# apollozkp/zkp-subnet

Measured on AMD Instinct MI355X. Metric: BLS12-381 G1 MSM points/sec at 2^20, higher is better.
Workload: dtype u32; 1 GPU; 2^20-point BLS12-381 G1 Pippenger MSM per GPU (uniform scalars in [0,r), cached SRS); points_per_gpu=1048576, window_bits=20, windows=13, buckets=524288, entries_per_lane=104, lanes=131072, requests_in_flight=1, world_size=1, parallelism=single GPU

## Files before the change

zkp_subnet_amd/csrc/msm.hip.h:

```cpp
#pragma once
#include "g1.hip.h"

struct WinLayout {
    int nwin;
    uint16_t off[66];
};
struct MsmShape {
    int c;
    int nwin;
    WinLayout lay;
    uint32_t nbuckets;
    uint64_t n;
    int nbatch;
    uint64_t srs_offset;
    uint64_t srs_stride;
    int chunk;
};

struct SortTail {
    uint32_t chunk;
    g1_xyzz_t* buckets;
    uint32_t* pin_dst;
    uint32_t* seq_word;
    uint32_t seq;
};
void launch_msm_sort(hipStream_t s, const MsmShape& sh, const uint32_t* scalars, int scalars_mont,
                     const uint32_t* scalars2, int scalars2_mont, uint32_t* part_ws, bool part_ws_clean, uint2* parted,
                     uint32_t* offsets, uint32_t* sorted, uint32_t* max_len_word, bool fast, uint32_t* overflow_word,
                     const SortTail* tail = nullptr);
bool msm_sort_fast_ok(const MsmShape& sh);
uint64_t msm_sort_parted_entries(const MsmShape& sh, bool fast);
void launch_publish(hipStream_t s, const void* src_dev, void* dst_host_devptr, uint32_t bytes, uint32_t* clear2 = nullptr,
                    uint32_t* seq_word_devptr = nullptr, uint32_t seq = 0);
void launch_msm_accumulate(hipStream_t s, const MsmShape& sh, const g1_affine_t* table, const uint32_t* offsets,
                           const uint32_t* sorted, g1_xyzz_t* buckets, g1_xyzz_t* carries, uint32_t* carry_key,
                           uint32_t nchunks);
void launch_fold_maxlen(hipStream_t s, const uint32_t* offsets, uint32_t nbuckets, uint32_t chunk, uint32_t* max_len,
                        g1_xyzz_t* buckets);
bool msm_fold_bucket_ok(uint32_t nbuckets, uint32_t max_run);
void launch_fold_bucket(hipStream_t s, const uint32_t* offsets, uint32_t chunk, uint32_t nbuckets, const g1_xyzz_t* carries,
                        g1_xyzz_t* buckets);
void launch_fold_step(hipStream_t s, const uint32_t* offsets, const uint32_t* carry_key, uint32_t chunk,
                      uint32_t nchunks, uint32_t d, g1_xyzz_t* carries);
void launch_fold_heads(hipStream_t s, const uint32_t* offsets, const uint32_t* carry_key, uint32_t chunk,
                       uint32_t nchunks, const g1_xyzz_t* carries, g1_xyzz_t* buckets);
void launch_msm_tree_level(hipStream_t s, const g1_xyzz_t* in, const g1_xyzz_t* prev, g1_xyzz_t* out,
                           uint32_t n_in_nodes, int level);
bool msm_tree_level2_ok(uint32_t n_in_nodes, int level);
void launch_msm_tree_level2(hipStream_t s, const g1_xyzz_t* in, const g1_xyzz_t* prev, g1_xyzz_t* mid_p, g1_xyzz_t* out,
                            uint32_t n_in_nodes, int level);
void launch_msm_final(hipStream_t s, const g1_xyzz_t* node, const g1_xyzz_t* prev, int nbits, int nodes,
                      g1_xyzz_t* out_xyzz, g1_xyzz_t* scratch);
void launch_g1_sum(hipStream_t s, const g1_xyzz_t* in, uint32_t count, g1_xyzz_t* out_xyzz);
void launch_g1_sum_affine(hipStream_t s, const g1_affine_t* in, uint32_t count, g1_xyzz_t* out_xyzz);
void launch_g1_subgroup_check(hipStream_t s, const g1_affine_t* in, uint32_t count, uint32_t* bad_flag);
void launch_g1_subgroup_check_bulk(hipStream_t s, const g1_affine_t* in, uint64_t n, uint32_t* bad_flag);
void launch_g1_compress(hipStream_t s, const g1_xyzz_t* in, uint8_t* out48);
void launch_g1_compress_pair(hipStream_t s, const g1_xyzz_t* in0, const g1_xyzz_t* in1, uint8_t* out0, uint8_t* out1);
void launch_xyzz_pack(hipStream_t s, const g1_xyzz_t* in, uint32_t* out48w, uint32_t count);
void launch_xyzz_unpack(hipStream_t s, const uint32_t* in48w, g1_xyzz_t* out, uint32_t count);

void launch_srs_from_be96(hipStream_t s, const uint8_t* be96, g1_affine_t* out, uint64_t n, uint32_t* bad_flag);
void launch_srs_from_c48(hipStream_t s, const uint8_t* c48, g1_affine_t* out, uint64_t n, uint32_t* bad_flag);
void launch_srs_to_c48(hipStream_t s, const g1_affine_t* in, uint8_t* c48, uint64_t n);
void launch_srs_to_be96(hipStream_t s, const g1_affine_t* in, uint8_t* be96, uint64_t n);
void launch_srs_precompute(hipStream_t s, g1_affine_t* table, uint64_t stride, uint64_t first, uint64_t count,
                           const WinLayout& lay, g1_xyzz_t* tmp);
void launch_srs_generate(hipStream_t s, g1_affine_t* out, uint64_t count, uint64_t j_base, const uint32_t* tau_mont,
                         const uint32_t* s0_mont, g1_affine_t* gtab, g1_xyzz_t* tmp, bool build_gtab);
```

zkp_subnet_amd/csrc/msm_tree.hip:

```cpp
#include "msm_dev.hip.h"

KZG_DEV void tree_operands(const g1_xyzz_t* in, const g1_xyzz_t* prev, uint32_t n_in, int level, uint32_t k, uint32_t m,
                           const g1_xyzz_t*& pa, const g1_xyzz_t*& pb) {
    if (level >= 1 && k == (uint32_t)level) {
        pa = &prev[4 * (uint64_t)m + 1];
        pb = &prev[4 * (uint64_t)m + 3];
    } else {
        pa = &in[(uint64_t)k * n_in + 2 * m];
        pb = pa + 1;
    }
}
#ifndef KZG_TREE_MIN_WAVES
#define KZG_TREE_MIN_WAVES 2
#endif
__global__ void __launch_bounds__(256, KZG_TREE_MIN_WAVES) k_msm_tree_level(const g1_xyzz_t* __restrict__ in,
                                                         const g1_xyzz_t* __restrict__ prev,
                                                         g1_xyzz_t* __restrict__ out, uint32_t n_in, int level) {
    tail_priority();
    const uint32_t n_out = n_in >> 1;
    const uint32_t gid = blockIdx.x * blockDim.x + threadIdx.x;
    if (gid >= n_out * (uint32_t)(level + 1)) return;
    const uint32_t k = gid / n_out, m = gid - k * n_out;
    const g1_xyzz_t *pa, *pb;
    tree_operands(in, prev, n_in, level, k, m, pa, pb);
    g1_xyzz_t a, b, r;
    load_xyzz(a, pa);
    load_xyzz(b, pb);
    g1_add<true>(r, a, b);
    if ((n_out & 63u) == 0) {
        __shared__ uint4 stage[4][64 * 15];
        const uint32_t lane = threadIdx.x & 63u;
        uint4* mine = stage[threadIdx.x >> 6];
        uint32_t t[56];
        const fp_t* f[4] = {&r.x, &r.y, &r.zz, &r.zzz};
#pragma unroll
        for (int c = 0; c < 4; c++)
#pragma unroll
            for (int i = 0; i < 14; i++) t[14 * c + i] = f[c]->l[i];
#pragma unroll
        for (int i = 0; i < 14; i++) mine[lane * 15 + i] = make_uint4(t[4 * i], t[4 * i + 1], t[4 * i + 2], t[4 * i + 3]);
        __builtin_amdgcn_fence(__ATOMIC_RELEASE, "wavefront");
        __builtin_amdgcn_wave_barrier();
        __builtin_amdgcn_fence(__ATOMIC_ACQUIRE, "wavefront");
        uint4* wb = reinterpret_cast<uint4*>(&out[(uint64_t)k * n_out + (m - lane)]);
#pragma unroll
        for (int i = 0; i < 14; i++) {
            const uint32_t g = (uint32_t)i * 64u + lane;
            const uint32_t pt = g / 14u;
            wb[g] = mine[pt * 15 + (g - pt * 14u)];
        }
        return;
    }
    store_xyzz(&out[(uint64_t)k * n_out + m], r);
}


__global__ void __launch_bounds__(256) k_msm_tree_level_coop(const g1_xyzz_t* __restrict__ in,
                                                              const g1_xyzz_t* __restrict__ prev,
                                                              g1_xyzz_t* __restrict__ out, uint32_t n_in, int level) {
    tail_priority();
    __shared__ CoopLds sm;
    const uint32_t n_out = n_in >> 1;
    const uint32_t gid = blockIdx.x * 64 + (threadIdx.x & 63);
    const bool active = gid < n_out * (uint32_t)(level + 1);
    const uint32_t k = active ? gid / n_out : 0, m = active ? gid - k * n_out : 0;
    const g1_xyzz_t *pa, *pb;
    tree_operands(in, prev, n_in, level, k, m, pa, pb);
    coop_add(sm, &out[(uint64_t)k * n_out + m], pa, pb, active);
}

__global__ void __launch_bounds__(64) k_msm_tree_level_lp(const g1_xyzz_t* __restrict__ in,
                                                           const g1_xyzz_t* __restrict__ prev,
                                                           g1_xyzz_t* __restrict__ out, uint32_t n_in, int level) {
    tail_priority();
    __shared__ LpScratch sm;
    const LpLane k = lp_lane();
    const uint32_t n_out = n_in >> 1;
    const uint32_t gid = blockIdx.x;
    const uint32_t c = gid / n_out, m = gid - c * n_out;
    const g1_xyzz_t *pa, *pb;
    tree_operands(in, prev, n_in, level, c, m, pa, pb);
    lp_add(sm, &out[(uint64_t)c * n_out + m], pa, pb, k);
}
__global__ void __launch_bounds__(128) k_msm_tree_level2_lp(const g1_xyzz_t* __restrict__ in,
                                                             const g1_xyzz_t* __restrict__ prev,
                                                             g1_xyzz_t* __restrict__ mid_p, g1_xyzz_t* __restrict__ out,
                                                             uint32_t n_in, int level) {
    tail_priority();
    __shared__ LpScratch sm[2];
    __shared__ __align__(16) g1_xyzz_t mid[2];
    const LpLane k = lp_lane();
    const uint32_t w = __builtin_amdgcn_readfirstlane(threadIdx.x >> 6);
    const uint32_t n2 = n_in >> 2;
    const uint32_t c = blockIdx.x / n2, j = blockIdx.x - c * n2;
    const bool late = c == (uint32_t)level + 1u;
    g1_xyzz_t* dst = &out[(uint64_t)c * n2 + j];
    if (late) {
        if (w == 0) lp_add(sm[0], dst, &in[4 * (uint64_t)j + 1], &in[4 * (uint64_t)j + 3], k);
    } else {
        const g1_xyzz_t *pa, *pb;
        tree_operands(in, prev, n_in, level, c, 2 * j + w, pa, pb);
        lp_add(sm[w], &mid[w], pa, pb, k);
    }
    __syncthreads();
    if (late) return;
    if (c == 0 && threadIdx.x < 112)
        reinterpret_cast<uint32_t*>(&mid_p[2 * (uint64_t)j])[threadIdx.x] = reinterpret_cast<const uint32_t*>(mid)[threadIdx.x];
    if (w == 0) lp_add(sm[0], dst, &mid[0], &mid[1], k);
}
#define FINAL_PTS 32
__global__ void __launch_bounds__(64) k_msm_final_dbl_lp(const g1_xyzz_t* __restrict__ node,
                                                          const g1_xyzz_t* __restrict__ prev, int nbits, int nodes,
                                                          g1_xyzz_t* __restrict__ pts) {
    tail_priority();
    __shared__ LpScratch sm;
    __shared__ g1_xyzz_t v;
    const LpLane k = lp_lane();
    const int l = (int)(blockIdx.x % (uint32_t)(nbits + 1));
    const uint32_t m = blockIdx.x / (uint32_t)(nbits + 1);
    const g1_xyzz_t* src = l < nbits - 1 ? &node[(uint64_t)(1 + l) * nodes + m] : l == nbits - 1 ? &prev[2 * m + 1] : &node[m];
    if (threadIdx.x < 56) reinterpret_cast<uint32_t*>(&v)[threadIdx.x] = reinterpret_cast<const uint32_t*>(src)[threadIdx.x];
    __syncthreads();
    if (l < nbits)
        for (int s = 0; s < l; s++) lp_dbl(sm, &v, &v, k);
    __syncthreads();
    if (threadIdx.x < 56)
        reinterpret_cast<uint32_t*>(&pts[(uint64_t)m * FINAL_PTS + l])[threadIdx.x] = reinterpret_cast<const uint32_t*>(&v)[threadIdx.x];
}
__global__ void __launch_bounds__(512) k_msm_final_sum_lp(const g1_xyzz_t* __restrict__ pts_g, int nbits,
                                                           g1_xyzz_t* __restrict__ out) {
    tail_priority();
    __shared__ LpScratch sm[8];
    __shared__ g1_xyzz_t pts[FINAL_PTS];
    const LpLane k = lp_lane();
    const int w = (int)__builtin_amdgcn_readfirstlane(threadIdx.x >> 6);
    const uint32_t m = blockIdx.x;
    const int count = nbits + 1;
    for (uint32_t i = threadIdx.x; i < (uint32_t)count * 56; i += 512)
        reinterpret_cast<uint32_t*>(pts)[i] = reinterpret_cast<const uint32_t*>(pts_g + (uint64_t)m * FINAL_PTS)[i];
    __syncthreads();
    for (int d = 16; d >= 1; d >>= 1) {
        for (int l = w; l < d; l += 8)
            if (l + d < count) lp_add(sm[w], &pts[l], &pts[l], &pts[l + d], k);
        __syncthreads();
    }
    if (threadIdx.x < 56) reinterpret_cast<uint32_t*>(&out[m])[threadIdx.x] = reinterpret_cast<const uint32_t*>(&pts[0])[threadIdx.x];
}


__global__ void __launch_bounds__(256) k_msm_final(const g1_xyzz_t* __restrict__ node,
                                                    const g1_xyzz_t* __restrict__ prev, int nbits, int nodes,
                                                    g1_xyzz_t* __restrict__ out) {
    tail_priority();
    __shared__ CoopLds sm;
    __shared__ g1_xyzz_t pts[64];
    const uint32_t l = threadIdx.x & 63;
    const uint32_t m = blockIdx.x;
    if (threadIdx.x < 64) {
        g1_xyzz_t v;
        g1_set_inf(v);
        if ((int)l < nbits - 1) load_xyzz(v, &node[(uint64_t)(1 + l) * nodes + m]);
        else if ((int)l == nbits - 1) load_xyzz(v, &prev[2 * m + 1]);
        else if ((int)l == nbits) load_xyzz(v, &node[m]);
        store_xyzz(&pts[l], v);
    }
    __syncthreads();
    for (int step = 0; step < nbits - 1; step++)
        coop_dbl(sm, &pts[l], &pts[l], (int)l < nbits && step < (int)l);
    for (uint32_t d = (nbits + 1 <= 32 ? 16 : 32); d >= 1; d >>= 1)
        coop_add(sm, &pts[l], &pts[l], &pts[l + d < 64 ? l + d : l], l < d);
    if (threadIdx.x == 0) {
        g1_xyzz_t v;
        load_xyzz(v, &pts[0]);
        store_xyzz(&out[m], v);
    }
}


#ifndef KZG_TREE_WIDE_MIN
#define KZG_TREE_WIDE_MIN 32768
#endif
void launch_msm_tree_level(hipStream_t s, const g1_xyzz_t* in, const g1_xyzz_t* prev, g1_xyzz_t* out,
                           uint32_t n_in_nodes, int level) {
    uint32_t ops = (n_in_nodes >> 1) * (uint32_t)(level + 1);
    if (ops > KZG_TREE_WIDE_MIN) k_msm_tree_level<<<nblk(ops, 256), 256, 0, s>>>(in, prev, out, n_in_nodes, level);
#ifndef KZG_NO_LP
    else if (ops <= LP_MAX_OPS) k_msm_tree_level_lp<<<ops, 64, 0, s>>>(in, prev, out, n_in_nodes, level);
#endif
    else k_msm_tree_level_coop<<<nblk(ops, 64), 256, 0, s>>>(in, prev, out, n_in_nodes, level);
}
bool msm_tree_level2_ok(uint32_t n_in_nodes, int level) {
#if defined(KZG_NO_LP) || defined(KZG_NO_TREE_PAIRS)
    (void)n_in_nodes; (void)level;
    return false;
#else
    return n_in_nodes >= 4 && (n_in_nodes >> 1) * (uint32_t)(level + 1) <= LP_MAX_OPS;
#endif
}
void launch_msm_tree_level2(hipStream_t s, const g1_xyzz_t* in, const g1_xyzz_t* prev, g1_xyzz_t* mid_p, g1_xyzz_t* out,
                            uint32_t n_in_nodes, int level) {
    k_msm_tree_level2_lp<<<(n_in_nodes >> 2) * (uint32_t)(level + 2), 128, 0, s>>>(in, prev, mid_p, out, n_in_nodes, level);
}
void launch_msm_final(hipStream_t s, const g1_xyzz_t* node, const g1_xyzz_t* prev, int nbits, int nodes,
                      g1_xyzz_t* out_xyzz, g1_xyzz_t* scratch) {
#ifndef KZG_NO_LP
    k_msm_final_dbl_lp<<<nodes * (nbits + 1), 64, 0, s>>>(node, prev, nbits, nodes, scratch);
    k_msm_final_sum_lp<<<nodes, 512, 0, s>>>(scratch, nbits, out_xyzz);
#else
    (void)scratch;
    k_msm_final<<<nodes, 256, 0, s>>>(node, prev, nbits, nodes, out_xyzz);
#endif
}
```

zkp_subnet_amd/csrc/pipeline.hip:

```cpp
#include "ctx.hip.h"

using namespace kzg_impl;

namespace kzg_impl {

#ifndef KZG_MIN_CHUNK
#define KZG_MIN_CHUNK 6
#endif
int pick_chunk(uint64_t entries) {
    const uint64_t lanes = 131072;
    if (entries <= lanes * 16) {
        const uint64_t k = (entries + lanes / 2 - 1) / (lanes / 2);
        return (int)(k < KZG_MIN_CHUNK ? KZG_MIN_CHUNK : k);
    }
    const uint64_t rounds = (entries + lanes * 512 - 1) / (lanes * 512);
    const uint64_t k = (entries + lanes * rounds - 1) / (lanes * rounds);
    return (int)k;
}
struct TreeBufs {
    g1_xyzz_t *in, *prev, *out, *extra;
};
static void run_tree(hipStream_t s, TreeBufs& b, uint32_t n_in, uint32_t stop) {
    for (int level = 0; n_in > stop;) {
        if ((n_in >> 2) >= stop && msm_tree_level2_ok(n_in, level)) {
            launch_msm_tree_level2(s, b.in, b.prev, b.out, b.extra, n_in, level);
            g1_xyzz_t *old_in = b.in, *old_prev = b.prev;
            b.in = b.extra;
            b.prev = b.out;
            b.out = old_prev;
            b.extra = old_in;
            level += 2;
            n_in >>= 2;
            continue;
        }
        launch_msm_tree_level(s, b.in, b.prev, b.out, n_in, level);
        g1_xyzz_t* recycled = b.prev;
        b.prev = b.in;
        b.in = b.out;
        b.out = recycled;
        level++;
        n_in >>= 1;
    }
}
int msm_core(kzg_ctx* ctx, Lane& L, const uint32_t* scalars, int mont, uint64_t n, uint64_t srs_offset,
             g1_xyzz_t* out_xyzz, const uint32_t* scalars2, int mont2) {
    hipStream_t s = L.stream;
    const int nbatch = scalars2 ? 2 : 1;
    if (n == 0) {
        HIPCHK(ctx, hipMemsetAsync(out_xyzz, 0, nbatch * sizeof(g1_xyzz_t), s));
        return KZG_OK;
    }
    if (srs_offset + n > ctx->stride) return fail(ctx, KZG_E_ARG, "MSM range exceeds the resident SRS");
    const uint64_t entries = n * (uint64_t)ctx->nwin * nbatch;
    if (entries >= ((uint64_t)1 << 32)) return fail(ctx, KZG_E_ARG, "MSM too large for 32-bit entry indices");
    MsmShape sh;
    sh.c = ctx->c; sh.nwin = ctx->nwin; sh.lay = ctx->lay; sh.nbuckets = ctx->nbuckets * nbatch; sh.n = n;
    sh.nbatch = nbatch;
    sh.srs_offset = srs_offset; sh.srs_stride = ctx->stride; sh.chunk = pick_chunk(entries);
    const uint32_t nchunks = (uint32_t)((entries + sh.chunk - 1) / sh.chunk);
    const size_t B = sh.nbuckets;
    L.expect_short = entries <= ((uint64_t)1 << 24);
    L.expect_us += 400 + (uint32_t)(entries / 4096);
    bool fast = msm_sort_fast_ok(sh) && L.skew_hint == 0;
    if (L.skew_hint > 0) L.skew_hint--;
    HIPCHK(ctx, L.rank.ensure(msm_sort_parted_entries(sh, msm_sort_fast_ok(sh)) * 8));
    HIPCHK(ctx, L.sorted.ensure(entries * 4));
    HIPCHK(ctx, L.hist.ensure(16384 * 4));
    HIPCHK(ctx, L.offsets.ensure((B + 1) * 4));
    HIPCHK(ctx, L.bufA.ensure(B * sizeof(g1_xyzz_t) + 16384));
    HIPCHK(ctx, L.bufB.ensure(B * sizeof(g1_xyzz_t) / 2 + 16384));
    HIPCHK(ctx, L.bufC.ensure(B * sizeof(g1_xyzz_t) / 2 + 16384));
    HIPCHK(ctx, L.bufD.ensure((size_t)(LP_MAX_OPS + 64) * sizeof(g1_xyzz_t) + 16384));
    HIPCHK(ctx, L.carries.ensure((size_t)nchunks * sizeof(g1_xyzz_t)));
    HIPCHK(ctx, L.carry_key.ensure((size_t)nchunks * 4));
    uint32_t* max_len_d = L.flags() + 2;
    uint32_t* max_len_h = reinterpret_cast<uint32_t*>(L.pin + PIN_MAXLEN);
    auto sort_and_publish = [&](bool fast_mode, bool ws_clean) {
        const SortTail tail{(uint32_t)sh.chunk, L.bufA.as<g1_xyzz_t>(), reinterpret_cast<uint32_t*>(L.pin_dev + PIN_MAXLEN),
                            reinterpret_cast<uint32_t*>(L.pin_dev + PIN_SEQ_SORT), ++L.sort_seq};
        launch_msm_sort(s, sh, scalars, mont, scalars2, mont2, L.hist.as<uint32_t>(), ws_clean, L.rank.as<uint2>(),
                        L.offsets.as<uint32_t>(), L.sorted.as<uint32_t>(), max_len_d, fast_mode, max_len_d + 1,
                        &tail);
    };
    {
        Span sp(ctx, L, KZG_T_DIGITS);
        sort_and_publish(fast, L.sort_ws_clean);
        L.sort_ws_clean = true;
        HIPCHK(ctx, hipEventRecord(L.ev_sorted, s));
    }
    {
        Span sp(ctx, L, KZG_T_ACCUMULATE);
        launch_msm_accumulate(s, sh, ctx->table.as<g1_affine_t>(), L.offsets.as<uint32_t>(), L.sorted.as<uint32_t>(),
                              L.bufA.as<g1_xyzz_t>(), L.carries.as<g1_xyzz_t>(), L.carry_key.as<uint32_t>(), nchunks);
    }
    auto wait_sorted = [&]() -> hipError_t {
#ifndef KZG_NO_POLL
        if (ctx->profiling != 1 && L.expect_short && poll_pinned(ctx, L, PIN_SEQ_SORT, L.sort_seq)) return hipSuccess;
#endif
        return hipEventSynchronize(L.ev_sorted);
    };
    HIPCHK(ctx, wait_sorted());
    if (fast && max_len_h[1]) {
        L.skew_hint = 16;
        {
            Span sp(ctx, L, KZG_T_DIGITS);
            sort_and_publish(false, true);
            HIPCHK(ctx, hipEventRecord(L.ev_sorted, s));
        }
        {
            Span sp(ctx, L, KZG_T_ACCUMULATE);
            launch_msm_accumulate(s, sh, ctx->table.as<g1_affine_t>(), L.offsets.as<uint32_t>(), L.sorted.as<uint32_t>(),
                                  L.bufA.as<g1_xyzz_t>(), L.carries.as<g1_xyzz_t>(), L.carry_key.as<uint32_t>(), nchunks);
        }
        HIPCHK(ctx, wait_sorted());
    }
    {
        Span sp(ctx, L, KZG_T_FIXUP);
        if (nchunks && msm_fold_bucket_ok(sh.nbuckets, *max_len_h)) {
            launch_fold_bucket(s, L.offsets.as<uint32_t>(), (uint32_t)sh.chunk, sh.nbuckets, L.carries.as<g1_xyzz_t>(),
                               L.bufA.as<g1_xyzz_t>());
        } else {
            for (uint32_t d = 1; d < *max_len_h; d <<= 1)
                launch_fold_step(s, L.offsets.as<uint32_t>(), L.carry_key.as<uint32_t>(), (uint32_t)sh.chunk, nchunks, d,
                                 L.carries.as<g1_xyzz_t>());
            launch_fold_heads(s, L.offsets.as<uint32_t>(), L.carry_key.as<uint32_t>(), (uint32_t)sh.chunk, nchunks,
                              L.carries.as<g1_xyzz_t>(), L.bufA.as<g1_xyzz_t>());
        }
    }
    TreeBufs tb{L.bufA.as<g1_xyzz_t>(), L.bufC.as<g1_xyzz_t>(), L.bufB.as<g1_xyzz_t>(), L.bufD.as<g1_xyzz_t>()};
    {
        Span sp(ctx, L, KZG_T_TREE);
        run_tree(s, tb, sh.nbuckets, (uint32_t)nbatch);
    }
    {
        Span sp(ctx, L, KZG_T_FINAL);
        launch_msm_final(s, tb.in, tb.prev, ctx->c - 1, nbatch, out_xyzz, tb.out);
    }
    HIPCHK(ctx, hipGetLastError());
    return KZG_OK;
}

int ensure_twiddles(kzg_ctx* ctx, Lane& L, int log_n, int inverse, uint32_t** tw, uint32_t** invn) {
    std::lock_guard<std::mutex> lk(ctx->mu);
    auto& m = inverse ? ctx->tw_inv : ctx->tw_fwd;
    bool built = false;
    if (log_n >= 1 && !m.count(log_n)) {
        DevBuf b;
        HIPCHK(ctx, b.ensure(((size_t)1 << (log_n - 1)) * 48));
        launch_fr_twiddles(L.stream, b.as<uint32_t>(), log_n, inverse);
        m[log_n] = std::move(b);
        built = true;
    }
    *tw = log_n >= 1 ? m[log_n].as<uint32_t>() : nullptr;
    if (invn) {
        if (!ctx->inv_n.count(log_n)) {
            DevBuf b;
            HIPCHK(ctx, b.ensure(32));
            launch_fr_inv_pow2(L.stream, b.as<uint32_t>(), log_n);
            ctx->inv_n[log_n] = std::move(b);
            built = true;
        }
        *invn = ctx->inv_n[log_n].as<uint32_t>();
    }
    if (built) HIPCHK(ctx, hipStreamSynchronize(L.stream));
    return KZG_OK;
}
int row_to_coeffs(kzg_ctx* ctx, Lane& L, const uint32_t* row_dev, uint64_t T, int evaluation_form, const uint32_t** coeffs,
                  uint32_t* dst) {
    if (!evaluation_form || T == 1) {
        if (dst && dst != row_dev) HIPCHK(ctx, hipMemcpyAsync(dst, row_dev, T * 32, hipMemcpyDeviceToDevice, L.stream));
        *coeffs = dst ? dst : row_dev;
        return KZG_OK;
    }
    int lg = ilog2_exact(T);
    if (lg < 0) return fail(ctx, KZG_E_ARG, "evaluation-form row length must be a power of two");
    uint32_t *tw, *invn;
    int rc = ensure_twiddles(ctx, L, lg, 1, &tw, &invn);
    if (rc) return rc;
    if (!dst) {
        HIPCHK(ctx, L.coeffB.ensure(T * 32));
        dst = L.coeffB.as<uint32_t>();
    }
    HIPCHK(ctx, L.ntt_mid.ensure(T * 48));
    Span sp(ctx, L, KZG_T_NTT);
    launch_fr_ntt(L.stream, row_dev, dst, lg, tw, invn, L.ntt_mid.as<uint32_t>());
    *coeffs = dst;
    return KZG_OK;
}
int check_worker(kzg_ctx* ctx, uint32_t i, uint64_t T) {
    int rc = need_srs(ctx);
    if (rc) return rc;
    if (T == 0) return fail(ctx, KZG_E_ARG, "empty polynomial");
    if (T > ctx->T) return fail(ctx, KZG_E_ARG, "polynomial longer than the worker's SRS slice");
    if ((uint64_t)i * ctx->T >= ctx->stride || (uint64_t)i * ctx->T + T > ctx->stride)
        return fail(ctx, KZG_E_ARG, "worker index outside the resident SRS");
    return KZG_OK;
}
const uint8_t* flushed_twin(kzg_ctx* ctx, const uint8_t* host_ptr, uint64_t bytes, hipEvent_t* ev) {
    for (Stage& st : ctx->stage)
        if (host_ptr && st.p_pub.load(std::memory_order_acquire) == host_ptr) {
            if (st.consumed_by && st.consumed_by != call_id_current()) {
                st.flushed = 0;
                return nullptr;
            }
            if (st.flushed >= bytes && st.flushed && st.twin.p) {
                st.consumed_by = call_id_current();
                *ev = st.ev;
                return static_cast<const uint8_t*>(st.twin.p);
            }
            return nullptr;
        }
    return nullptr;
}
int upload_fr(kzg_ctx* ctx, Lane& L, const uint8_t* be32, uint64_t n, uint32_t* dst, int to_mont) {
    if (!n) return KZG_OK;
    Span sp(ctx, L, KZG_T_DECODE);
    hipEvent_t ev = nullptr;
    if (const uint8_t* twin = flushed_twin(ctx, be32, n * 32, &ev)) {
        HIPCHK(ctx, hipStreamWaitEvent(L.stream, ev, 0));
        L.in_be_src = twin;
    } else {
        HIPCHK(ctx, L.in_be.ensure(n * 32));
        HIPCHK(ctx, hipMemcpyAsync(L.in_be.p, be32, n * 32, hipMemcpyHostToDevice, L.stream));
        L.in_be_src = L.in_be.as<uint8_t>();
    }
    launch_fr_from_be(L.stream, L.in_be_src, dst, n, to_mont, L.flags());
    return KZG_OK;
}


#ifndef KZG_BATCHED_ROW_MAX
#define KZG_BATCHED_ROW_MAX ((uint64_t)1 << 18)
#endif
int commit_open_dev(kzg_ctx* ctx, LaneHold& H, uint32_t i, const uint32_t* row_dev, uint64_t T, int evaluation_form,
                    const uint8_t* alpha_be32, uint8_t* out_c48, uint8_t* out_eval32, uint8_t* out_p48,
                    const uint32_t* coeffs_ready, uint32_t* coeffs_dst, const VerifyJob* verify) {
    Lane& A = H.L();
    hipStream_t s = A.stream;
    const uint32_t* coeffs = coeffs_ready;
    int rc = KZG_OK;
    if (!coeffs) rc = row_to_coeffs(ctx, A, row_dev, T, evaluation_form, &coeffs, coeffs_dst);
    if (rc) return rc;
    const uint64_t offset = (uint64_t)i * ctx->T;
    g1_xyzz_t* res = A.res();
    const bool both = out_c48 && out_p48;
    const bool batched = both && T <= KZG_BATCHED_ROW_MAX;
    Lane* B = (both && !batched) ? H.second() : nullptr;
    Lane& O = B ? *B : A;
    hipStream_t so = O.stream;
    if (B) {
        HIPCHK(ctx, hipEventRecord(A.ev_coeffs, s));
        HIPCHK(ctx, hipStreamWaitEvent(so, A.ev_coeffs, 0));
    }
    if (out_c48 && !batched) {
        rc = msm_core(ctx, A, coeffs, 1, T, offset, res);
        if (rc) return rc;
    }
    if (out_p48) {
        uint32_t* alpha_m = reinterpret_cast<uint32_t*>(A.tail + TB_ALPHA_M);
        uint32_t* y_m = reinterpret_cast<uint32_t*>(A.tail + TB_Y_M);
        const uint64_t nchunks = (T + 3) / 4;
        HIPCHK(ctx, O.hbuf.ensure((nchunks + (nchunks >> 1) + 64) * 32));
        HIPCHK(ctx, O.hnext.ensure((nchunks + (nchunks >> 1) + 64) * 32));
        HIPCHK(ctx, O.qbuf.ensure(T * 32));
        {
            Span sp(ctx, A, KZG_T_POLY, so);
            launch_poly_open(so, coeffs, T, alpha_m, O.hbuf.as<uint32_t>(), O.hnext.as<uint32_t>(), y_m,
                             O.qbuf.as<uint32_t>(), alpha_be32, A.flags(), A.tail + TB_EVAL);
        }
        if (batched) {
            rc = msm_core(ctx, A, coeffs, 1, T, offset, res, O.qbuf.as<uint32_t>(), 0);
        } else {
            rc = msm_core(ctx, O, O.qbuf.as<uint32_t>(), 0, T - 1, offset, res + 1);
        }
        if (rc) return rc;
        if (B) {
            HIPCHK(ctx, hipEventRecord(B->ev_done, so));
            HIPCHK(ctx, hipStreamWaitEvent(s, B->ev_done, 0));
        }
    }
    queue_encode(ctx, A, out_c48 != nullptr, out_p48 != nullptr);
    if (verify) {
        uint32_t* vflag = reinterpret_cast<uint32_t*>(A.tail + TB_VERIFY);
        HIPCHK(ctx, hipMemsetAsync(vflag, 0, 4, A.vstream));
        hipEvent_t fev = nullptr;
        const uint32_t* mine = reinterpret_cast<const uint32_t*>(flushed_twin(ctx, verify->row_be32, verify->T * 32, &fev));
        if (mine) {
            HIPCHK(ctx, hipStreamWaitEvent(A.vstream, fev, 0));
        } else {
            HIPCHK(ctx, A.vbuf.ensure(verify->T * 32));
            HIPCHK(ctx, hipMemcpyAsync(A.vbuf.p, verify->row_be32, verify->T * 32, hipMemcpyHostToDevice, A.vstream));
            mine = A.vbuf.as<uint32_t>();
        }
        launch_words_differ(A.vstream, mine, verify->cached_raw, verify->T * 8, vflag);
        HIPCHK(ctx, hipEventRecord(A.ev_verify, A.vstream));
        HIPCHK(ctx, hipStreamWaitEvent(s, A.ev_verify, 0));
    }
    rc = finish(ctx, A);
    if (rc) return rc;
    if (out_c48 && out_p48 && ctx->host_finish)
        kzg_host::xyzz_pair_to_c48(reinterpret_cast<const uint32_t*>(A.pin + TB_RES0),
                                   reinterpret_cast<const uint32_t*>(A.pin + TB_RES1), out_c48, out_p48);
    else {
        if (out_c48) result_c48(ctx, A, 0, out_c48);
        if (out_p48) result_c48(ctx, A, 1, out_p48);
    }
    if (out_p48) memcpy(out_eval32, A.pin + TB_EVAL, 32);
    H.clean = true;
    return KZG_OK;
}

}
```

Before: 399.7 million points/s.

## Fuse up to three bucket-tree reduction levels into one block-local kernel

Adds a kernel that runs several consecutive levels of the bucket reduction tree inside one launch, with each block reducing its own slice and using __syncthreads between levels. The host tree driver now uses this fused path for the wide early levels, rotating output buffers through five slots that include the two halves of the input buffer. bufD is enlarged to hold half the buckets for this purpose. The aim is to cut kernel launches and inter-level gaps on the widest levels, at the cost of idle threads as later levels shrink and extra scratch memory.

```diff
diff --git a/zkp_subnet_amd/csrc/msm.hip.h b/zkp_subnet_amd/csrc/msm.hip.h
--- a/zkp_subnet_amd/csrc/msm.hip.h
+++ b/zkp_subnet_amd/csrc/msm.hip.h
@@ -46,6 +46,9 @@
                        uint32_t nchunks, const g1_xyzz_t* carries, g1_xyzz_t* buckets);
 void launch_msm_tree_level(hipStream_t s, const g1_xyzz_t* in, const g1_xyzz_t* prev, g1_xyzz_t* out,
                            uint32_t n_in_nodes, int level);
+int msm_tree_sub_levels(uint32_t n_in_nodes, int level, uint32_t stop);
+void launch_msm_tree_sub(hipStream_t s, const g1_xyzz_t* in, const g1_xyzz_t* prev, g1_xyzz_t* const* outs,
+                         uint32_t n_in_nodes, int level, int nlev);
 bool msm_tree_level2_ok(uint32_t n_in_nodes, int level);
 void launch_msm_tree_level2(hipStream_t s, const g1_xyzz_t* in, const g1_xyzz_t* prev, g1_xyzz_t* mid_p, g1_xyzz_t* out,
                             uint32_t n_in_nodes, int level);
diff --git a/zkp_subnet_amd/csrc/msm_tree.hip b/zkp_subnet_amd/csrc/msm_tree.hip
--- a/zkp_subnet_amd/csrc/msm_tree.hip
+++ b/zkp_subnet_amd/csrc/msm_tree.hip
@@ -9,6 +9,34 @@
         pa = &in[(uint64_t)k * n_in + 2 * m];
         pb = pa + 1;
     }
+}
+KZG_DEV void tree_store(g1_xyzz_t* __restrict__ out, uint32_t n_out, uint32_t k, uint32_t m, const g1_xyzz_t& r,
+                        bool staged) {
+    if (staged) {
+        __shared__ uint4 stage[4][64 * 15];
+        const uint32_t lane = threadIdx.x & 63u;
+        uint4* mine = stage[threadIdx.x >> 6];
+        uint32_t t[56];
+        const fp_t* f[4] = {&r.x, &r.y, &r.zz, &r.zzz};
+#pragma unroll
+        for (int c = 0; c < 4; c++)
+#pragma unroll
+            for (int i = 0; i < 14; i++) t[14 * c + i] = f[c]->l[i];
+#pragma unroll
+        for (int i = 0; i < 14; i++) mine[lane * 15 + i] = make_uint4(t[4 * i], t[4 * i + 1], t[4 * i + 2], t[4 * i + 3]);
+        __builtin_amdgcn_fence(__ATOMIC_RELEASE, "wavefront");
+        __builtin_amdgcn_wave_barrier();
+        __builtin_amdgcn_fence(__ATOMIC_ACQUIRE, "wavefront");
+        uint4* wb = reinterpret_cast<uint4*>(&out[(uint64_t)k * n_out + (m - lane)]);
+#pragma unroll
+        for (int i = 0; i < 14; i++) {
+            const uint32_t g = (uint32_t)i * 64u + lane;
+            const uint32_t pt = g / 14u;
+            wb[g] = mine[pt * 15 + (g - pt * 14u)];
+        }
+        return;
+    }
+    store_xyzz(&out[(uint64_t)k * n_out + m], r);
 }
 #ifndef KZG_TREE_MIN_WAVES
 #define KZG_TREE_MIN_WAVES 2
@@ -27,31 +55,39 @@
     load_xyzz(a, pa);
     load_xyzz(b, pb);
     g1_add<true>(r, a, b);
-    if ((n_out & 63u) == 0) {
-        __shared__ uint4 stage[4][64 * 15];
-        const uint32_t lane = threadIdx.x & 63u;
-        uint4* mine = stage[threadIdx.x >> 6];
-        uint32_t t[56];
-        const fp_t* f[4] = {&r.x, &r.y, &r.zz, &r.zzz};
-#pragma unroll
-        for (int c = 0; c < 4; c++)
-#pragma unroll
-            for (int i = 0; i < 14; i++) t[14 * c + i] = f[c]->l[i];
-#pragma unroll
-        for (int i = 0; i < 14; i++) mine[lane * 15 + i] = make_uint4(t[4 * i], t[4 * i + 1], t[4 * i + 2], t[4 * i + 3]);
-        __builtin_amdgcn_fence(__ATOMIC_RELEASE, "wavefront");
-        __builtin_amdgcn_wave_barrier();
-        __builtin_amdgcn_fence(__ATOMIC_ACQUIRE, "wavefront");
-        uint4* wb = reinterpret_cast<uint4*>(&out[(uint64_t)k * n_out + (m - lane)]);
-#pragma unroll
-        for (int i = 0; i < 14; i++) {
-            const uint32_t g = (uint32_t)i * 64u + lane;
-            const uint32_t pt = g / 14u;
-            wb[g] = mine[pt * 15 + (g - pt * 14u)];
+    tree_store(out, n_out, k, m, r, (n_out & 63u) == 0);
+}
+
+#define TREE_SUB_MAX 3
+struct TreeSubOuts {
+    g1_xyzz_t* p[TREE_SUB_MAX];
+};
+__global__ void __launch_bounds__(256, KZG_TREE_MIN_WAVES) k_msm_tree_sub(const g1_xyzz_t* __restrict__ in,
+                                                                          const g1_xyzz_t* __restrict__ prev,
+                                                                          TreeSubOuts outs, uint32_t n_in, int level,
+                                                                          int nlev, uint32_t cnt) {
+    tail_priority();
+    const g1_xyzz_t* cur = in;
+    const g1_xyzz_t* below = prev;
+#pragma unroll 1
+    for (int j = 0; j < nlev; j++, level++, n_in >>= 1, cnt >>= 1) {
+        const uint32_t n_out = n_in >> 1;
+        const uint32_t ops = cnt * (uint32_t)(level + 1);
+        g1_xyzz_t* out = outs.p[j];
+        if (threadIdx.x < ops) {
+            const uint32_t k = threadIdx.x / cnt, m = blockIdx.x * cnt + (threadIdx.x - k * cnt);
+            const g1_xyzz_t *pa, *pb;
+            tree_operands(cur, below, n_in, level, k, m, pa, pb);
+            g1_xyzz_t a, b, r;
+            load_xyzz(a, pa);
+            load_xyzz(b, pb);
+            g1_add<true>(r, a, b);
+            tree_store(out, n_out, k, m, r, (cnt & 63u) == 0);
         }
-        return;
-    }
-    store_xyzz(&out[(uint64_t)k * n_out + m], r);
+        if (j + 1 < nlev) __syncthreads();
+        below = cur;
+        cur = out;
+    }
 }
 
 
@@ -189,6 +225,25 @@
 #endif
     else k_msm_tree_level_coop<<<nblk(ops, 64), 256, 0, s>>>(in, prev, out, n_in_nodes, level);
 }
+#ifndef KZG_TREE_SUB_LEVELS
+#define KZG_TREE_SUB_LEVELS 3
+#endif
+static_assert(KZG_TREE_SUB_LEVELS >= 1 && KZG_TREE_SUB_LEVELS <= TREE_SUB_MAX, "KZG_TREE_SUB_LEVELS out of range");
+int msm_tree_sub_levels(uint32_t n_in_nodes, int level, uint32_t stop) {
+    int w = 0;
+    for (uint32_t n = n_in_nodes; w < KZG_TREE_SUB_LEVELS && (n >> 1) >= stop && (n >> 1) * (uint32_t)(level + w + 1) > KZG_TREE_WIDE_MIN;
+         n >>= 1)
+        w++;
+    return w >= 2 ? w : 0;
+}
+void launch_msm_tree_sub(hipStream_t s, const g1_xyzz_t* in, const g1_xyzz_t* prev, g1_xyzz_t* const* outs,
+                         uint32_t n_in_nodes, int level, int nlev) {
+    uint32_t cnt = 256;
+    while (cnt * (uint32_t)(level + 1) > 256) cnt >>= 1;
+    TreeSubOuts o{};
+    for (int j = 0; j < nlev; j++) o.p[j] = outs[j];
+    k_msm_tree_sub<<<(n_in_nodes >> 1) / cnt, 256, 0, s>>>(in, prev, o, n_in_nodes, level, nlev, cnt);
+}
 bool msm_tree_level2_ok(uint32_t n_in_nodes, int level) {
 #if defined(KZG_NO_LP) || defined(KZG_NO_TREE_PAIRS)
     (void)n_in_nodes; (void)level;
diff --git a/zkp_subnet_amd/csrc/pipeline.hip b/zkp_subnet_amd/csrc/pipeline.hip
--- a/zkp_subnet_amd/csrc/pipeline.hip
+++ b/zkp_subnet_amd/csrc/pipeline.hip
@@ -21,7 +21,29 @@
     g1_xyzz_t *in, *prev, *out, *extra;
 };
 static void run_tree(hipStream_t s, TreeBufs& b, uint32_t n_in, uint32_t stop) {
-    for (int level = 0; n_in > stop;) {
+    int level = 0;
+    if (int nlev = msm_tree_sub_levels(n_in, level, stop)) {
+        g1_xyzz_t* const lo = b.in;
+        g1_xyzz_t* const hi = b.in + n_in / 2;
+        g1_xyzz_t* const slot[5] = {b.out, b.prev, b.extra, lo, hi};
+        for (; nlev; nlev = msm_tree_sub_levels(n_in, level, stop)) {
+            g1_xyzz_t* outs[3];
+            int k = 0;
+            for (g1_xyzz_t* p : slot) {
+                const bool busy = level == 0 ? (p == lo || p == hi) : (p == b.in || p == b.prev);
+                if (!busy && k < nlev) outs[k++] = p;
+            }
+            launch_msm_tree_sub(s, b.in, b.prev, outs, n_in, level, nlev);
+            b.prev = nlev >= 2 ? outs[nlev - 2] : b.in;
+            b.in = outs[nlev - 1];
+            level += nlev;
+            n_in >>= nlev;
+        }
+        int k = 0;
+        for (g1_xyzz_t* p : slot)
+            if (p != b.in && p != b.prev && k < 2) (k++ ? b.extra : b.out) = p;
+    }
+    while (n_in > stop) {
         if ((n_in >> 2) >= stop && msm_tree_level2_ok(n_in, level)) {
             launch_msm_tree_level2(s, b.in, b.prev, b.out, b.extra, n_in, level);
             g1_xyzz_t *old_in = b.in, *old_prev = b.prev;
@@ -70,7 +92,8 @@
     HIPCHK(ctx, L.bufA.ensure(B * sizeof(g1_xyzz_t) + 16384));
     HIPCHK(ctx, L.bufB.ensure(B * sizeof(g1_xyzz_t) / 2 + 16384));
     HIPCHK(ctx, L.bufC.ensure(B * sizeof(g1_xyzz_t) / 2 + 16384));
-    HIPCHK(ctx, L.bufD.ensure((size_t)(LP_MAX_OPS + 64) * sizeof(g1_xyzz_t) + 16384));
+    const size_t d_pts = msm_tree_sub_levels((uint32_t)B, 0, (uint32_t)nbatch) ? B / 2 : 0;
+    HIPCHK(ctx, L.bufD.ensure(std::max(d_pts, (size_t)LP_MAX_OPS + 64) * sizeof(g1_xyzz_t) + 16384));
     HIPCHK(ctx, L.carries.ensure((size_t)nchunks * sizeof(g1_xyzz_t)));
     HIPCHK(ctx, L.carry_key.ensure((size_t)nchunks * 4));
     uint32_t* max_len_d = L.flags() + 2;
```

Measured after the change: 400.8 million points/s (median of 6 runs). Within noise of the previous version (+0.3%).

## Fuse carry fold and first two tree levels into one bucket-tree kernel

Applied to the files above, without the earlier changes.

Adds a kernel that folds per-chunk carries into buckets for its 1024-bucket block, then computes the first two bucket-reduction tree levels from groups of four buckets, writing odd partials and two output rows. A companion launch runs level 2 with a compact odd-prev layout before the regular tree continues at level 3. The aim is to drop the separate fixup launch and one tree-level pass over the 2^19 buckets, which saves launches and global memory round-trips. In exchange, each thread holds more work and does more LDS staging, and the carry fold is done serially inside each block.

```diff
diff --git a/zkp_subnet_amd/csrc/msm.hip.h b/zkp_subnet_amd/csrc/msm.hip.h
--- a/zkp_subnet_amd/csrc/msm.hip.h
+++ b/zkp_subnet_amd/csrc/msm.hip.h
@@ -46,6 +46,11 @@
                        uint32_t nchunks, const g1_xyzz_t* carries, g1_xyzz_t* buckets);
 void launch_msm_tree_level(hipStream_t s, const g1_xyzz_t* in, const g1_xyzz_t* prev, g1_xyzz_t* out,
                            uint32_t n_in_nodes, int level);
+bool msm_tree_first_ok(uint32_t nbuckets);
+void launch_msm_tree_first(hipStream_t s, g1_xyzz_t* buckets, const uint32_t* offsets, const uint32_t* carry_key,
+                           const g1_xyzz_t* carries, uint32_t chunk, uint32_t nbuckets, g1_xyzz_t* odd, g1_xyzz_t* out);
+void launch_msm_tree_level_after_first(hipStream_t s, const g1_xyzz_t* in, const g1_xyzz_t* odd, g1_xyzz_t* out,
+                                       uint32_t n_in_nodes);
 bool msm_tree_level2_ok(uint32_t n_in_nodes, int level);
 void launch_msm_tree_level2(hipStream_t s, const g1_xyzz_t* in, const g1_xyzz_t* prev, g1_xyzz_t* mid_p, g1_xyzz_t* out,
                             uint32_t n_in_nodes, int level);
diff --git a/zkp_subnet_amd/csrc/msm_tree.hip b/zkp_subnet_amd/csrc/msm_tree.hip
--- a/zkp_subnet_amd/csrc/msm_tree.hip
+++ b/zkp_subnet_amd/csrc/msm_tree.hip
@@ -1,10 +1,10 @@
 #include "msm_dev.hip.h"
 
 KZG_DEV void tree_operands(const g1_xyzz_t* in, const g1_xyzz_t* prev, uint32_t n_in, int level, uint32_t k, uint32_t m,
-                           const g1_xyzz_t*& pa, const g1_xyzz_t*& pb) {
+                           const g1_xyzz_t*& pa, const g1_xyzz_t*& pb, bool prev_odd = false) {
     if (level >= 1 && k == (uint32_t)level) {
-        pa = &prev[4 * (uint64_t)m + 1];
-        pb = &prev[4 * (uint64_t)m + 3];
+        pa = prev_odd ? &prev[2 * (uint64_t)m] : &prev[4 * (uint64_t)m + 1];
+        pb = prev_odd ? pa + 1 : &prev[4 * (uint64_t)m + 3];
     } else {
         pa = &in[(uint64_t)k * n_in + 2 * m];
         pb = pa + 1;
@@ -13,16 +13,37 @@
 #ifndef KZG_TREE_MIN_WAVES
 #define KZG_TREE_MIN_WAVES 2
 #endif
+KZG_DEV void store_xyzz_wave_run(uint4* mine, uint32_t lane, g1_xyzz_t* run, const g1_xyzz_t& r) {
+    uint32_t t[56];
+    const fp_t* f[4] = {&r.x, &r.y, &r.zz, &r.zzz};
+#pragma unroll
+    for (int c = 0; c < 4; c++)
+#pragma unroll
+        for (int i = 0; i < 14; i++) t[14 * c + i] = f[c]->l[i];
+#pragma unroll
+    for (int i = 0; i < 14; i++) mine[lane * 15 + i] = make_uint4(t[4 * i], t[4 * i + 1], t[4 * i + 2], t[4 * i + 3]);
+    __builtin_amdgcn_fence(__ATOMIC_RELEASE, "wavefront");
+    __builtin_amdgcn_wave_barrier();
+    __builtin_amdgcn_fence(__ATOMIC_ACQUIRE, "wavefront");
+    uint4* wb = reinterpret_cast<uint4*>(run);
+#pragma unroll
+    for (int i = 0; i < 14; i++) {
+        const uint32_t g = (uint32_t)i * 64u + lane;
+        const uint32_t pt = g / 14u;
+        wb[g] = mine[pt * 15 + (g - pt * 14u)];
+    }
+}
 __global__ void __launch_bounds__(256, KZG_TREE_MIN_WAVES) k_msm_tree_level(const g1_xyzz_t* __restrict__ in,
                                                          const g1_xyzz_t* __restrict__ prev,
-                                                         g1_xyzz_t* __restrict__ out, uint32_t n_in, int level) {
+                                                         g1_xyzz_t* __restrict__ out, uint32_t n_in, int level,
+                                                         int prev_odd) {
     tail_priority();
     const uint32_t n_out = n_in >> 1;
     const uint32_t gid = blockIdx.x * blockDim.x + threadIdx.x;
     if (gid >= n_out * (uint32_t)(level + 1)) return;
     const uint32_t k = gid / n_out, m = gid - k * n_out;
     const g1_xyzz_t *pa, *pb;
-    tree_operands(in, prev, n_in, level, k, m, pa, pb);
+    tree_operands(in, prev, n_in, level, k, m, pa, pb, prev_odd != 0);
     g1_xyzz_t a, b, r;
     load_xyzz(a, pa);
     load_xyzz(b, pb);
@@ -30,28 +51,56 @@
     if ((n_out & 63u) == 0) {
         __shared__ uint4 stage[4][64 * 15];
         const uint32_t lane = threadIdx.x & 63u;
-        uint4* mine = stage[threadIdx.x >> 6];
-        uint32_t t[56];
-        const fp_t* f[4] = {&r.x, &r.y, &r.zz, &r.zzz};
-#pragma unroll
-        for (int c = 0; c < 4; c++)
-#pragma unroll
-            for (int i = 0; i < 14; i++) t[14 * c + i] = f[c]->l[i];
-#pragma unroll
-        for (int i = 0; i < 14; i++) mine[lane * 15 + i] = make_uint4(t[4 * i], t[4 * i + 1], t[4 * i + 2], t[4 * i + 3]);
-        __builtin_amdgcn_fence(__ATOMIC_RELEASE, "wavefront");
-        __builtin_amdgcn_wave_barrier();
-        __builtin_amdgcn_fence(__ATOMIC_ACQUIRE, "wavefront");
-        uint4* wb = reinterpret_cast<uint4*>(&out[(uint64_t)k * n_out + (m - lane)]);
-#pragma unroll
-        for (int i = 0; i < 14; i++) {
-            const uint32_t g = (uint32_t)i * 64u + lane;
-            const uint32_t pt = g / 14u;
-            wb[g] = mine[pt * 15 + (g - pt * 14u)];
+        store_xyzz_wave_run(stage[threadIdx.x >> 6], lane, &out[(uint64_t)k * n_out + (m - lane)], r);
+        return;
+    }
+    store_xyzz(&out[(uint64_t)k * n_out + m], r);
+}
+
+#define TREE_FIRST_BUCKETS 1024u
+__global__ void __launch_bounds__(256, KZG_TREE_MIN_WAVES) k_msm_tree_first(g1_xyzz_t* __restrict__ buckets,
+                                                         const uint32_t* __restrict__ offsets,
+                                                         const uint32_t* __restrict__ carry_key,
+                                                         const g1_xyzz_t* __restrict__ carries, uint32_t chunk,
+                                                         uint32_t n_in, g1_xyzz_t* __restrict__ odd,
+                                                         g1_xyzz_t* __restrict__ out) {
+    tail_priority();
+    const uint32_t b_lo = blockIdx.x * TREE_FIRST_BUCKETS;
+    if (chunk) {
+        const uint32_t e_lo = offsets[b_lo], e_hi = offsets[min(b_lo + TREE_FIRST_BUCKETS, n_in)];
+        for (uint32_t c = e_lo / chunk + 1u + threadIdx.x; (uint64_t)c * chunk < e_hi; c += 256u) {
+            const uint32_t key = carry_key[c];
+            if (key == NONE_KEY) continue;
+            g1_xyzz_t a, b, r;
+            load_xyzz(a, &buckets[key]);
+            load_xyzz(b, &carries[c]);
+            g1_add<true>(r, a, b);
+            store_xyzz(&buckets[key], r);
         }
-        return;
-    }
-    store_xyzz(&out[(uint64_t)k * n_out + m], r);
+        __syncthreads();
+    }
+    __shared__ uint4 stage[4][64 * 15];
+    const uint32_t n_out = n_in >> 2;
+    const uint32_t lane = threadIdx.x & 63u;
+    const uint32_t w0 = __builtin_amdgcn_readfirstlane(blockIdx.x * blockDim.x + (threadIdx.x & ~63u));
+    uint4* mine = stage[threadIdx.x >> 6];
+    const g1_xyzz_t* b = &buckets[4 * (uint64_t)w0] + 4 * lane;
+    g1_xyzz_t x, y, r;
+    load_xyzz(x, b + 2);
+    load_xyzz(y, b + 3);
+    g1_add<true>(r, x, y);
+    store_xyzz_wave_run(mine, lane, &odd[w0], r);
+    load_xyzz(x, b);
+    load_xyzz(y, b + 1);
+    g1_add<true>(r, x, y);
+    __asm__ volatile("" ::: "memory");
+    load_xyzz(y, reinterpret_cast<const g1_xyzz_t*>(&mine[lane * 15]));
+    g1_add<true>(x, r, y);
+    store_xyzz_wave_run(mine, lane, &out[w0], x);
+    load_xyzz(x, b + 1);
+    load_xyzz(y, b + 3);
+    g1_add<true>(r, x, y);
+    store_xyzz_wave_run(mine, lane, &out[n_out + w0], r);
 }
 
 
@@ -183,11 +232,27 @@
 void launch_msm_tree_level(hipStream_t s, const g1_xyzz_t* in, const g1_xyzz_t* prev, g1_xyzz_t* out,
                            uint32_t n_in_nodes, int level) {
     uint32_t ops = (n_in_nodes >> 1) * (uint32_t)(level + 1);
-    if (ops > KZG_TREE_WIDE_MIN) k_msm_tree_level<<<nblk(ops, 256), 256, 0, s>>>(in, prev, out, n_in_nodes, level);
+    if (ops > KZG_TREE_WIDE_MIN) k_msm_tree_level<<<nblk(ops, 256), 256, 0, s>>>(in, prev, out, n_in_nodes, level, 0);
 #ifndef KZG_NO_LP
     else if (ops <= LP_MAX_OPS) k_msm_tree_level_lp<<<ops, 64, 0, s>>>(in, prev, out, n_in_nodes, level);
 #endif
     else k_msm_tree_level_coop<<<nblk(ops, 64), 256, 0, s>>>(in, prev, out, n_in_nodes, level);
+}
+void launch_msm_tree_level_after_first(hipStream_t s, const g1_xyzz_t* in, const g1_xyzz_t* odd, g1_xyzz_t* out,
+                                       uint32_t n_in_nodes) {
+    const uint32_t ops = (n_in_nodes >> 1) * 3u;
+    k_msm_tree_level<<<nblk(ops, 256), 256, 0, s>>>(in, odd, out, n_in_nodes, 2, 1);
+}
+#ifndef KZG_TREE_FIRST_MIN
+#define KZG_TREE_FIRST_MIN 131072
+#endif
+bool msm_tree_first_ok(uint32_t nbuckets) {
+    return (nbuckets >> 2) >= KZG_TREE_FIRST_MIN && nbuckets % TREE_FIRST_BUCKETS == 0;
+}
+void launch_msm_tree_first(hipStream_t s, g1_xyzz_t* buckets, const uint32_t* offsets, const uint32_t* carry_key,
+                           const g1_xyzz_t* carries, uint32_t chunk, uint32_t nbuckets, g1_xyzz_t* odd, g1_xyzz_t* out) {
+    k_msm_tree_first<<<nbuckets / TREE_FIRST_BUCKETS, 256, 0, s>>>(buckets, offsets, carry_key, carries, chunk, nbuckets,
+                                                                   odd, out);
 }
 bool msm_tree_level2_ok(uint32_t n_in_nodes, int level) {
 #if defined(KZG_NO_LP) || defined(KZG_NO_TREE_PAIRS)
diff --git a/zkp_subnet_amd/csrc/pipeline.hip b/zkp_subnet_amd/csrc/pipeline.hip
--- a/zkp_subnet_amd/csrc/pipeline.hip
+++ b/zkp_subnet_amd/csrc/pipeline.hip
@@ -20,8 +20,8 @@
 struct TreeBufs {
     g1_xyzz_t *in, *prev, *out, *extra;
 };
-static void run_tree(hipStream_t s, TreeBufs& b, uint32_t n_in, uint32_t stop) {
-    for (int level = 0; n_in > stop;) {
+static void run_tree(hipStream_t s, TreeBufs& b, uint32_t n_in, uint32_t stop, int level = 0) {
+    while (n_in > stop) {
         if ((n_in >> 2) >= stop && msm_tree_level2_ok(n_in, level)) {
             launch_msm_tree_level2(s, b.in, b.prev, b.out, b.extra, n_in, level);
             g1_xyzz_t *old_in = b.in, *old_prev = b.prev;
@@ -114,7 +114,9 @@
         }
         HIPCHK(ctx, wait_sorted());
     }
-    {
+    const bool tree_first = msm_tree_first_ok(sh.nbuckets);
+    const bool fold_in_tree = tree_first && nchunks && *max_len_h <= 1;
+    if (!fold_in_tree) {
         Span sp(ctx, L, KZG_T_FIXUP);
         if (nchunks && msm_fold_bucket_ok(sh.nbuckets, *max_len_h)) {
             launch_fold_bucket(s, L.offsets.as<uint32_t>(), (uint32_t)sh.chunk, sh.nbuckets, L.carries.as<g1_xyzz_t>(),
@@ -130,7 +132,15 @@
     TreeBufs tb{L.bufA.as<g1_xyzz_t>(), L.bufC.as<g1_xyzz_t>(), L.bufB.as<g1_xyzz_t>(), L.bufD.as<g1_xyzz_t>()};
     {
         Span sp(ctx, L, KZG_T_TREE);
-        run_tree(s, tb, sh.nbuckets, (uint32_t)nbatch);
+        if (tree_first) {
+            launch_msm_tree_first(s, tb.in, L.offsets.as<uint32_t>(), L.carry_key.as<uint32_t>(), L.carries.as<g1_xyzz_t>(),
+                                  fold_in_tree ? (uint32_t)sh.chunk : 0u, sh.nbuckets, tb.prev, tb.out);
+            launch_msm_tree_level_after_first(s, tb.out, tb.prev, tb.in, sh.nbuckets >> 2);
+            tb = TreeBufs{tb.in, tb.out, tb.prev, tb.extra};
+            run_tree(s, tb, sh.nbuckets >> 3, (uint32_t)nbatch, 3);
+        } else {
+            run_tree(s, tb, sh.nbuckets, (uint32_t)nbatch);
+        }
     }
     {
         Span sp(ctx, L, KZG_T_FINAL);
```

New measurement: 399.2 million points/s before, 401.7 million points/s after, median of 6. Within noise of the previous version (+0.6%).
